# mkaspr/Vulcan

Measured on AMD Instinct MI355X. Metric: RGB-D frames/sec (integrate+raycast), 640x480 @ 5 mm voxels, higher is better.
Workload: dtype f32

## Files before the change

vulcan_amd/csrc/vk_common.hpp:

```cpp
#pragma once

#include <hip/hip_runtime.h>
#include <stdint.h>
#include <float.h>

#include "../../include/vk.h"

#define VK_CHECK(expr)                                  \
  do {                                                  \
    const hipError_t vk_e__ = (expr);                   \
    if (vk_e__ != hipSuccess)                           \
    {                                                   \
      (void)hipGetLastError();                          \
      return (int)vk_e__;                               \
    }                                                   \
  } while (0)

#define VK_REQUIRE(cond)                                \
  do {                                                  \
    if (!(cond)) return VK_ERR_ARGUMENT;                \
  } while (0)

#ifdef VK_DEBUG_SYNC
#define VK_LAUNCH_CHECK()                               \
// ... 157 lines not shown
  int16_t ox, oy, oz, pad;
  int32_t data;
  int32_t next;
};
static_assert(sizeof(Entry) == 16, "HashEntry layout");

__device__ __forceinline__ Entry load_entry(const vk_hash_entry* entries, uint32_t index)
{
  const int4 raw = reinterpret_cast<const int4*>(entries)[index];
  Entry e;
  e.ox = (int16_t)(raw.x & 0xffff);
  e.oy = (int16_t)((uint32_t)raw.x >> 16);
  e.oz = (int16_t)(raw.y & 0xffff);
  e.pad = (int16_t)((uint32_t)raw.y >> 16);
  e.data = raw.z;
  e.next = raw.w;
  return e;
}

__device__ __forceinline__ bool entry_is(const Entry& e, int bx, int by, int bz)
{
  return e.ox == (int16_t)bx && e.oy == (int16_t)by && e.oz == (int16_t)bz;
}

__device__ __forceinline__ int lane_id() { return (int)(threadIdx.x & 63); }

__device__ __forceinline__ void wave_lds_fence()
{
  __builtin_amdgcn_fence(__ATOMIC_RELEASE, "wavefront");
  __builtin_amdgcn_wave_barrier();
  __builtin_amdgcn_fence(__ATOMIC_ACQUIRE, "wavefront");
}


template <typename K>
__device__ __forceinline__ f3 normal_from_taps(const K& k, int x, int y, float depth,
    float left, float right, float up, float down)
{
  const int pad = 2;
  f3 normal = make3(0, 0, 0);
  if (depth > 0)
  {
    const f3 z0 = unproject_d(k, (x + 0) + 0.5f, (y + 0) + 0.5f, depth);
    const f3 x0 = (left == 0) ? z0 : scale3(unproject(k, (x - pad) + 0.5f, (y + 0) + 0.5f), left);
    const f3 x1 = (right == 0) ? z0 : scale3(unproject(k, (x + pad) + 0.5f, (y + 0) + 0.5f), right);
    const f3 y0 = (up == 0) ? z0 : scale3(unproject(k, (x + 0) + 0.5f, (y - pad) + 0.5f), up);
    const f3 y1 = (down == 0) ? z0 : scale3(unproject(k, (x + 0) + 0.5f, (y + pad) + 0.5f), down);
    const f3 dx = sub3(x0, x1);
    const f3 dy = sub3(y0, y1);
    if (sqnorm3(dx) > 0 && sqnorm3(dy) > 0) normal = normalized3(cross3(dy, dx));
  }
  return normal;
}

template <typename Load>
__device__ __forceinline__ float depth_or_zero(Load load, int w, int h, int x, int y)
{
  return (x >= 0 && x < w && y >= 0 && y < h) ? load(y * w + x) : 0.0f;
}

template <typename K, typename Load>
__device__ __forceinline__ f3 pixel_normal(const K& k, Load load, int w, int h, int x, int y, float depth)
{
  const int pad = 2;
  f3 normal = make3(0, 0, 0);
  if (depth > 0)
// ... 32 lines not shown
```

vulcan_amd/csrc/vk_requests.hpp:

```cpp
#pragma once

#include "vk_common.hpp"

#include <string.h>

namespace vk
{

__device__ __forceinline__ unsigned long long request_key(int type, int bx, int by, int bz)
{
  return ((unsigned long long)(uint16_t)type << 48) | ((unsigned long long)(uint16_t)(int16_t)bz << 32) |
         ((unsigned long long)(uint16_t)(int16_t)by << 16) | (unsigned long long)(uint16_t)(int16_t)bx;
}

constexpr uint8_t kTouched = 4;
__device__ __forceinline__ uint32_t band_tag(int y, int height)
{
  int band = (int)(((long long)y * VK_BANDS) / (height > 0 ? height : 1));
  band = band < 0 ? 0 : (band >= VK_BANDS ? VK_BANDS - 1 : band);
  return (uint32_t)(band + 1) << 3;
}

enum { MARK_PLAIN = 0, MARK_DEFER = 1, MARK_APPEND = 2 };

// ... 25 lines not shown
{
  return reinterpret_cast<unsigned long long*>(counters + VK_CTR_PUBLIC) + (size_t)which * VK_RETRY_SLOTS;
}
__host__ __device__ inline int* retry_slots(int32_t* counters, int which)
{
  return counters + VK_CTR_PUBLIC + 2 * 2 * VK_RETRY_SLOTS + which * VK_RETRY_KEYS;
}

__host__ __device__ inline int* posted_list(int32_t* counters)
{
  return counters + VK_CTR_PUBLIC + 2 * 2 * VK_RETRY_SLOTS + 2 * VK_RETRY_KEYS;
}
constexpr uint32_t kPostedExcess = 0x80000000u;
constexpr uint32_t kPostedBucket = 0x7fffffffu;

struct Retry
{
  int* contended;
  int* origin_seen;
  int* count;
  int* overflow;
  unsigned long long* table;
  int* slots;
  int capacity;
  int* posted;
  int* posted_tail;
  int* posted_count;
  int posted_capacity;
};

__device__ __forceinline__ void file_loser(const Retry& retry, unsigned long long key)
{
  uint32_t at = (uint32_t)((key * 0x9E3779B97F4A7C15ull) >> 40) & (uint32_t)(VK_RETRY_SLOTS - 1);
  for (int tries = 0; tries < 64; ++tries)
  {
    const unsigned long long old = atomicCAS(retry.table + at, 0ull, key);
    if (old == key) return;
    if (old == 0ull)
    {
      const int n = atomicAdd(retry.count, 1);
      if (n < retry.capacity) retry.slots[n] = (int)at;
      else __hip_atomic_store(retry.overflow, 1, __ATOMIC_RELAXED, __HIP_MEMORY_SCOPE_AGENT);
      return;
    }
    at = (at + 1) & (uint32_t)(VK_RETRY_SLOTS - 1);
  }
  __hip_atomic_store(retry.overflow, 1, __ATOMIC_RELAXED, __HIP_MEMORY_SCOPE_AGENT);
}

__device__ __forceinline__ void post_request(const vk_volume& v, uint32_t h, int type, int bx, int by, int bz,
    const Retry& retry, uint32_t tail)
{
  unsigned long long* slot = reinterpret_cast<unsigned long long*>(v.allocation_blocks) + h;
  const unsigned long long key = request_key(type, bx, by, bz);
  unsigned long long seen = __hip_atomic_load(slot, __ATOMIC_RELAXED, __HIP_MEMORY_SCOPE_AGENT);
  if (seen < key) seen = atomicMax(slot, key);
  if (retry.contended)
  {
    if (seen != 0ull && seen != key)
    {
      file_loser(retry, seen < key ? seen : key);
      if (__hip_atomic_load(retry.contended, __ATOMIC_RELAXED, __HIP_MEMORY_SCOPE_AGENT) == 0)
        __hip_atomic_store(retry.contended, 1, __ATOMIC_RELAXED, __HIP_MEMORY_SCOPE_AGENT);
    }
    if (seen == 0ull && retry.posted)
    {
// ... 27 lines not shown
  else
  {
    bool found = false;
    uint32_t index = hash_code;

    for (int guard = 0; entry.next != -1 && guard < v.excess_block_count; ++guard)
    {
      index = (uint32_t)entry.next;
      entry = load_entry(v.hash_entries, index);

      if (entry_is(entry, bx, by, bz))
      {
        mark_visible<MARK>(v, index, -1, tag);
        found = true;
        break;
      }
    }

    if (!found) post_request(v, hash_code, VK_ALLOC_EXCESS, bx, by, bz, retry, index);
  }
}

__device__ __forceinline__ int left_lane(int v)
{
  return __builtin_amdgcn_update_dpp(v, v, 0x138, 0xf, 0xf, false);
}

constexpr int kVisitSlots = 96;
constexpr int kVisitWords = 3 * kVisitSlots;
constexpr int kVisitWalkCap = 6 + 4096;

struct RequestParams
{
  vk_volume v;
  const float* depth;
  int width, height;
  Projection k;
  Rt Twd;
  const float* colors;
  const float* normals;
  Rt Tcd;
  float depth_threshold;
  float* mask;
  float4* records;
  float* normals_out;
};

template <int MARK>
__device__ __forceinline__ void request_walk(const RequestParams& P, int x, int y, const Retry& retry, int* visits)
{
  const vk_volume& v = P.v;
  const uint32_t K = (uint32_t)v.main_block_count;
  const float block_length = VK_BLOCK_RESOLUTION * v.voxel_length;
  const float truncation_length = v.truncation_length;
  const uint32_t tag = MARK == MARK_DEFER ? band_tag(y, P.height) : 0u;

  f3 direction = unproject(P.k, x + 0.5f, y + 0.5f);
  direction = xform_dir(P.Twd, direction);
  const f3 origin = make3(P.Twd.r[3], P.Twd.r[7], P.Twd.r[11]);

  float depth = 0.0f;
  if (x < P.width) depth = P.depth[y * P.width + x];
  const bool usable = x < P.width && !(depth < v.min_depth || depth > v.max_depth);

  const f3 Xwp = add3(origin, scale3(direction, depth));
  direction = normalized3(direction);
  const f3 begin = sub3(Xwp, scale3(direction, truncation_length));
  const f3 end = add3(Xwp, scale3(direction, truncation_length));

  const int step_x = (direction.x < 0) ? -1 : 1;
  const int step_y = (direction.y < 0) ? -1 : 1;
  const int step_z = (direction.z < 0) ? -1 : 1;

  const float inv_block_length = 1.0f / block_length;
  int bx = f2i(floorf(begin.x * inv_block_length));
  int by = f2i(floorf(begin.y * inv_block_length));
  int bz = f2i(floorf(begin.z * inv_block_length));
  const int ex = f2i(floorf(end.x * inv_block_length));
  const int ey = f2i(floorf(end.y * inv_block_length));
  const int ez = f2i(floorf(end.z * inv_block_length));

  const float ox = block_length * (bx + vmaxi(0, step_x)) - begin.x;
  const float oy = block_length * (by + vmaxi(0, step_y)) - begin.y;
  const float oz = block_length * (bz + vmaxi(0, step_z)) - begin.z;

  float tmax_x = ox / direction.x;
  float tmax_y = oy / direction.y;
  float tmax_z = oz / direction.z;
  if (direction.x == 0) tmax_x = (float)1E20;
  if (direction.y == 0) tmax_y = (float)1E20;
  if (direction.z == 0) tmax_z = (float)1E20;

  const float tdelta_x = (step_x * block_length) / direction.x;
  const float tdelta_y = (step_y * block_length) / direction.y;
  const float tdelta_z = (step_z * block_length) / direction.z;

  int* const list_x = visits;
  int* const list_y = visits + kVisitSlots;
  int* const list_z = visits + 2 * kVisitSlots;
  const int lane = lane_id();
  bool walking = usable;
  int listed = 0;

  for (int step = 0;; ++step)
  {
    const bool left_walking = left_lane((int)walking) != 0;
    const int left_x = left_lane(bx), left_y = left_lane(by), left_z = left_lane(bz);
    const bool fresh = walking && !(lane > 0 && left_walking && left_x == bx && left_y == by && left_z == bz);
    const unsigned long long fresh_mask = __ballot(fresh);
    const int arriving = __popcll(fresh_mask);
    const bool last = arriving == 0;

    if (listed + arriving > kVisitSlots || last)
    {
      wave_lds_fence();
      for (int first = 0; first < listed; first += 64)
      {
        const int at = first + lane;
        if (at < listed)
        {
          const int px = list_x[at], py = list_y[at], pz = list_z[at];
          const uint32_t hash_code = block_hash(px, py, pz, K);
          const Entry entry = load_entry(v.hash_entries, hash_code);
          const uint8_t byte = v.block_visibility[hash_code];
          probe_block<MARK>(v, hash_code, entry, px, py, pz, retry, (int)byte, tag);
        }
      }
      wave_lds_fence();
      listed = 0;
    }
    if (last) break;

    if (fresh)
    {
      const int at = listed + (int)__builtin_amdgcn_mbcnt_hi((uint32_t)(fresh_mask >> 32),
          __builtin_amdgcn_mbcnt_lo((uint32_t)fresh_mask, 0u));
      list_x[at] = bx; list_y[at] = by; list_z[at] = bz;
    }
    listed += arriving;

    if (walking)
    {
      if (tmax_x < tmax_y)
      {
        if (tmax_x < tmax_z) { bx += step_x; if (bx == ex + step_x) walking = false; else tmax_x += tdelta_x; }
        else                 { bz += step_z; if (bz == ez + step_z) walking = false; else tmax_z += tdelta_z; }
      }
      else
      {
        if (tmax_y < tmax_z) { by += step_y; if (by == ey + step_y) walking = false; else tmax_y += tdelta_y; }
        else                 { bz += step_z; if (bz == ez + step_z) walking = false; else tmax_z += tdelta_z; }
      }
      if (step + 1 >= kVisitWalkCap) walking = false;
    }
  }
}

template <int PREP>
struct RequestLds
{
  static constexpr int HALO = (PREP == 2) ? 2 : 1;
  static constexpr int TW = 69 + HALO, TH = 9 + HALO, TS = 72;
  static constexpr int kTileWords = PREP ? TH * TS : 0, kRowWords = PREP ? 2 * 10 * 64 : 0;
  static constexpr int kListWords = 4 * kVisitWords;
  static constexpr int kAreaWords = kTileWords + (kRowWords > kListWords ? kRowWords : kListWords);
  static constexpr int kBytes = 4 * kAreaWords;
  static_assert(!PREP || kListWords <= kRowWords, "the visit lists lie over row_min / row_max");
};
constexpr int kLdsPerCU = 160 * 1024;
constexpr int kRequestGroupsPerCU = 6;
static_assert(kRequestGroupsPerCU * RequestLds<0>::kBytes <= kLdsPerCU && kRequestGroupsPerCU * RequestLds<1>::kBytes <= kLdsPerCU &&
    kRequestGroupsPerCU * RequestLds<2>::kBytes <= kLdsPerCU, "LDS of the request pass at six workgroups per CU");

template <bool DEFER, int PREP>
__device__ __forceinline__ void requests_group(const RequestParams P, const Retry retry, const int group_x, const int group_y)
{
  const int x = group_x * 64 + (int)(threadIdx.x & 63);
  const int y = group_y * 4 + (int)(threadIdx.x >> 6);
  if (DEFER && group_x == 0 && group_y == 0 && threadIdx.x < VK_BANDS) band_counts(P.v.counters)[threadIdx.x] = 0;

  using L = RequestLds<PREP>;
  constexpr int HALO = L::HALO, TW = L::TW, TH = L::TH, TS = L::TS;
  constexpr int LOADS = (TW * TH + 255) / 256;
  __shared__ int area[L::kAreaWords];
  float* const tile = reinterpret_cast<float*>(area);
  float* const row_min = reinterpret_cast<float*>(area + L::kTileWords);
  float* const row_max = row_min + 10 * 64;
  int* const visits = area + L::kTileWords + (int)(threadIdx.x >> 6) * kVisitWords;
  float staged[LOADS] = {};
  vf3 prep_rgb = {0.0f, 0.0f, 0.0f}, prep_n = {0.0f, 0.0f, 0.0f};
  if (PREP)
  {
    const int x0 = group_x * 64 - HALO, y0 = group_y * 4 - HALO;
#pragma unroll
    for (int t = 0; t < LOADS; ++t)
    {
      const int i = (int)threadIdx.x + 256 * t;
      const int r = i / TW, c = i - r * TW;
      const int vx = x0 + c, vy = y0 + r;
      if (i < TW * TH && vx >= 0 && vx < P.width && vy >= 0 && vy < P.height) staged[t] = P.depth[vy * P.width + vx];
    }
    if (x < P.width && y < P.height)
    {
      const int index = y * P.width + x;
      prep_rgb = *reinterpret_cast<const vf3*>(P.colors + 3 * (size_t)index);
      if (PREP == 1) prep_n = *reinterpret_cast<const vf3*>(P.normals + 3 * (size_t)index);
    }
  }

  if (y < P.height) request_walk<DEFER ? MARK_DEFER : MARK_PLAIN>(P, x, y, retry, visits);

  if (PREP)
  {
#pragma unroll
    for (int t = 0; t < LOADS; ++t)
    {
      const int i = (int)threadIdx.x + 256 * t;
      if (i < TW * TH) tile[(i / TW) * TS + (i % TW)] = staged[t];
    }
    __syncthreads();
#pragma unroll
    for (int t = 0; t < 3; ++t)
    {
      const int e = (int)threadIdx.x + 256 * t;
      if (e < 10 * 64)
      {
        const float* at = tile + (HALO - 1 + (e >> 6)) * TS + (HALO + 2 + (e & 63));
        float lo = +FLT_MAX, hi = -FLT_MAX;
#pragma unroll
        for (int j = -3; j <= 3; ++j)
        {
          lo = fminf(at[j], lo);
          hi = fmaxf(at[j], hi);
        }
        row_min[e] = lo;
        row_max[e] = hi;
      }
    }
    __syncthreads();
    if (x < P.width && y < P.height)
    {
      const int index = y * P.width + x;
      const int lx = (int)(threadIdx.x & 63) + HALO, ly = (int)(threadIdx.x >> 6) + HALO;
      f3 normal = make3(prep_n.x, prep_n.y, prep_n.z);
      if (PREP == 2)
      {
        normal = normal_from_taps(P.k, x, y, tile[ly * TS + lx], tile[ly * TS + lx - 2], tile[ly * TS + lx + 2],
            tile[(ly - 2) * TS + lx], tile[(ly + 2) * TS + lx]);
        P.normals_out[3 * (size_t)index + 0] = normal.x;
        P.normals_out[3 * (size_t)index + 1] = normal.y;
        P.normals_out[3 * (size_t)index + 2] = normal.z;
      }
      const f3 Xcn = xform_dir(P.Tcd, normal);
      float m = 0.0f;
      if (light_color_usable(prep_rgb.x, prep_rgb.y, prep_rgb.z))
      {
        const int first = (int)(threadIdx.x >> 6) * 64 + (int)(threadIdx.x & 63);
        float dmin = +FLT_MAX, dmax = -FLT_MAX;
#pragma unroll
        for (int i = 0; i < 7; ++i)
        {
          dmin = fminf(row_min[first + 64 * i], dmin);
          dmax = fmaxf(row_max[first + 64 * i], dmax);
        }
        m = (dmax - dmin <= P.depth_threshold) ? 1.0f : 0.0f;
      }
      P.mask[index] = m;
      P.records[index] = make_float4(Xcn.x, Xcn.y, Xcn.z, m);
    }
  }
}


constexpr int kArrivalMaxWorkgroups = 65535;

inline int posted_capacity()
{
  const int n = vk_hook(VK_HOOK_POSTED_CAPACITY);
  return (n >= 0 && n < VK_POSTED_SLOTS) ? n : VK_POSTED_SLOTS;
}

inline int retry_capacity()
{
  const int n = vk_hook(VK_HOOK_RETRY_CAPACITY);
  return (n > 0 && n < VK_RETRY_KEYS) ? n : VK_RETRY_KEYS;
}

inline bool set_view_unfused(const vk_volume* v)
{
  const bool unfused = vk_hook(VK_HOOK_SET_VIEW_UNFUSED) == 1;
  return unfused || ((long long)v->main_block_count + v->excess_block_count) / 1024 + 16 > kArrivalMaxWorkgroups;
}

inline bool prep_rides(const vk_light_prep* prep, const vk_frame* frame)
{
  return prep && prep->mask && prep->records && frame->color && frame->normals && frame->content_id != 0 &&
      (long long)frame->width * frame->height <= (long long)prep->capacity &&
      (reinterpret_cast<uintptr_t>(prep->records) & 15) == 0 &&
      (frame->color_width <= 0 || frame->color_width == frame->width) &&
      (frame->color_height <= 0 || frame->color_height == frame->height);
}

inline void prep_note_made(vk_light_prep* prep, const vk_frame* frame)
{
  prep->depth = frame->depth;
  prep->color = frame->color;
  prep->normals = frame->normals;
  prep->width = frame->width;
  prep->height = frame->height;
  prep->depth_to_color = frame->depth_to_color;
  prep->content_id = frame->content_id;
  prep->prepared_threshold = prep->depth_threshold;
  prep->valid = 1;
  prep->normals_out = nullptr;
}

inline int build_request_pass(RequestParams& P, Retry& retry, const vk_volume* v, const float* depth, int width, int height,
    const vk_projection* projection, const vk_transform* Twd, const vk_frame* prep_frame, const vk_light_prep* prep, bool fused)
{
  P.v = *v;
  P.depth = depth;
  P.width = width;
  P.height = height;
  P.k = make_projection(*projection);
  P.Twd = make_rt(Twd->m);
  P.colors = P.normals = nullptr;
  P.Tcd = P.Twd;
  P.depth_threshold = 0.0f;
  P.mask = nullptr;
  P.records = nullptr;
  P.normals_out = nullptr;
  memset(&retry, 0, sizeof(retry));
  if (fused)
  {
    retry.contended = v->counters + VK_CTR_CONTENDED;
    retry.origin_seen = v->counters + VK_CTR_ORIGIN_SEEN;
    retry.count = v->counters + VK_CTR_RETRY_COUNT;
    retry.overflow = v->counters + VK_CTR_RETRY_OVERFLOW;
    retry.table = retry_table(v->counters, 0);
    retry.slots = retry_slots(v->counters, 0);
    retry.capacity = retry_capacity();
    if (!set_view_unfused(v))
    {
      retry.posted = posted_list(v->counters);
      retry.posted_tail = posted_list(v->counters) + VK_POSTED_SLOTS;
      retry.posted_count = v->counters + VK_CTR_POSTED;
      retry.posted_capacity = posted_capacity();
    }
  }
  if (!(prep && prep_frame)) return 0;
  P.colors = prep_frame->color;
  P.normals = prep_frame->normals;
  P.Tcd = make_rt(prep_frame->depth_to_color.m);
  P.depth_threshold = prep->depth_threshold;
  P.mask = prep->mask;
  P.records = reinterpret_cast<float4*>(prep->records);
  P.normals_out = prep->normals_out;
  return prep->normals_out ? 2 : 1;
}

}
```

vulcan_amd/csrc/vk_trace.hip:

```cpp
#include "vk_bounds.hpp"
#include "vk_raycast.hpp"
#include "vk_requests.hpp"

using namespace vk;

namespace
{


constexpr int kPatchThreads = 256;

__global__ __launch_bounds__(kPatchThreads) void compute_patches_kernel(PatchParams P)
{
  __shared__ int wave_total[kPatchThreads / 64];
  __shared__ int block_base;

  const int block_count = P.block_count_dev ? min(*P.block_count_dev, P.block_count) : P.block_count;
  const int index = blockIdx.x * kPatchThreads + threadIdx.x;
  const int lane = lane_id();
  const int wave = threadIdx.x >> 6;

  BlockRect r;
  r.count = 0;
  r.gx = r.gy = 0;
// ... 236 lines not shown
{
  if (threadIdx.x == 0)
  {
    const int first = vmaxi(group_y * 4 - 2, 0) >> 3, last = vmini(group_y * 4 + 5, P.image_height - 1) >> 3;
    int polls = 0;
    bool late = false;
    for (int row = first; row <= last && !late; ++row)
      while ((int)(__hip_atomic_load(&P.rows_done[row * kNormalRowStride], __ATOMIC_RELAXED, __HIP_MEMORY_SCOPE_AGENT) - P.rows_target) < 0)
      {
        if (++polls > P.normal_polls) { late = true; break; }
        __builtin_amdgcn_s_sleep(32);
      }
    *expired = late ? 1 : 0;
    if (late)
    {
      __hip_atomic_store(P.late_dev, P.late_tag, __ATOMIC_RELAXED, __HIP_MEMORY_SCOPE_AGENT);
      if (P.late_host) __hip_atomic_store(P.late_host, (int32_t)P.late_tag, __ATOMIC_RELAXED, __HIP_MEMORY_SCOPE_SYSTEM);
    }
  }
  __syncthreads();
  if (*expired) return;
  const int x = group_x * 64 + (threadIdx.x & 63);
  const int y = group_y * 4 + (threadIdx.x >> 6);
  if (x >= P.image_width || y >= P.image_height) return;
  const auto written = [depths = P.depths](int i) { return __hip_atomic_load(&depths[i], __ATOMIC_RELAXED, __HIP_MEMORY_SCOPE_AGENT); };
  const f3 normal = pixel_normal(P.k, written, P.image_width, P.image_height, x, y,
      depth_or_zero(written, P.image_width, P.image_height, x, y));
  const int output = y * P.image_width + x;
  normals[3 * output + 0] = normal.x;
  normals[3 * output + 1] = normal.y;
  normals[3 * output + 2] = normal.z;
}

template <bool POOL32, int PREP>
__global__ __launch_bounds__(256) __attribute__((amdgpu_waves_per_eu(VK_TR_WAVES))) void trace_and_request_kernel(PointParams P,
    RequestParams R, Retry retry, int trace_groups, int request_groups_x, int request_groups, float* normals)
{
  __shared__ int4 directories[4][kDirWords];
  __shared__ int normals_expired;
  static_assert(kRequestGroupsPerCU * (int)(sizeof(directories) + sizeof(int) + RequestLds<PREP>::kBytes) <= kLdsPerCU,
      "LDS of the raycast + request launch at six workgroups per CU");
  if ((int)blockIdx.x < trace_groups)
  {
    __builtin_amdgcn_s_setprio(2);
    points_group<POOL32, 4>(P, (int)blockIdx.x, trace_groups, directories);
    return;
  }
  const int g = (int)blockIdx.x - trace_groups;
  if (g < request_groups)
  {
    requests_group<true, PREP>(R, retry, g % request_groups_x, g / request_groups_x);
    return;
  }
  const int n = g - request_groups, normal_groups_x = (P.image_width + 63) / 64;
  normals_group(P, normals, n % normal_groups_x, n / normal_groups_x, &normals_expired);
}


__global__ __launch_bounds__(256) void compute_normals_kernel(const float* __restrict__ depths,
    vk_projection k, float* __restrict__ normals, int image_width, int image_height)
{
  const int x = blockIdx.x * 64 + (threadIdx.x & 63);
  const int y = blockIdx.y * 4 + (threadIdx.x >> 6);
  if (x >= image_width || y >= image_height) return;

  const f3 normal = pixel_normal(k, plain_depths{depths}, image_width, image_height, x, y, depths[y * image_width + x]);

  const int output = y * image_width + x;
  normals[3 * output + 0] = normal.x;
  normals[3 * output + 1] = normal.y;
  normals[3 * output + 2] = normal.z;
}

__global__ __launch_bounds__(256) void filter_depths_kernel(int image_width, int image_height,
    const float* __restrict__ src, float* __restrict__ dst)
{
  const int x = blockIdx.x * 64 + (threadIdx.x & 63);
  const int y = blockIdx.y * 4 + (threadIdx.x >> 6);
  if (x >= image_width || y >= image_height) return;

  const int pad = 3;
  const float d0 = src[y * image_width + x];
  float dn = 0;
  float w = 0;

  for (int i = -pad; i <= pad; ++i)
// ... 18 lines not shown
{
  const int cells = P.bounds_width * P.bounds_height;

  if (partials && cells <= kBoundsMaxCells)
  {
    hipLaunchKernelGGL(block_bounds_partial_kernel, dim3(kBoundsGroups), dim3(kBoundsThreads), 0, s, P, partials);
    VK_LAUNCH_CHECK();
    if (merge)
    {
      hipLaunchKernelGGL(merge_bounds_kernel, dim3((cells + 255) / 256), dim3(256), 0, s, partials,
          reinterpret_cast<float2*>(bounds), cells);
      VK_LAUNCH_CHECK();
    }
    return VK_OK;
  }

  hipLaunchKernelGGL(reset_bounds_kernel, dim3((cells + 255) / 256), dim3(256), 0, s,
      reinterpret_cast<float2*>(bounds), cells);
  VK_LAUNCH_CHECK();
  if (P.block_count == 0) return VK_OK;
  P.bounds = bounds;
  int blocks = (P.block_count + 255) / 256;
  if (blocks > kCUs * 4) blocks = kCUs * 4;
  hipLaunchKernelGGL(block_bounds_kernel, dim3(blocks), dim3(256), 0, s, P);
  VK_LAUNCH_CHECK();
  return VK_OK;
}

int launch_points(const vk_hash_entry* entries, const vk_voxel* voxels, const float* bounds,
    const float2* partials, int block_count, float block_length, float voxel_length, float trunc_length,
    const vk_transform* Twc, const vk_projection* projection, float* depths, float* colors,
    int image_width, int image_height, int bounds_width, int bounds_height, unsigned long long pool_bytes,
    hipStream_t s, float* normals = nullptr, uint32_t* rows_done = nullptr, uint32_t rows_target = 0,
    const RequestParams* next_requests = nullptr, const Retry* next_retry = nullptr, int next_prep = 0,
    int32_t* late_host = nullptr, int normal_polls = kNormalWaitPolls, uint32_t late_tag = 1)
{
  PointParams P;
  P.late_tag = late_tag ? late_tag : 1u;
  P.entries = entries;
  P.voxels = voxels;
  P.bounds = bounds;
  P.partials = partials;
  P.bounds_out = reinterpret_cast<float2*>(const_cast<float*>(bounds));
  P.K = (uint32_t)block_count;
  P.block_length = block_length;
  P.voxel_length = voxel_length;
  P.trunc_length = trunc_length;
  P.inv_block_length = 1.0 / (double)block_length;
  P.inv_voxel_length = 1.0 / (double)voxel_length;
  P.touched = nullptr;
  P.march_steps = nullptr;
  P.trip_log = nullptr;
  P.trip_log_passes = 0;
  P.rows_done = (normals && rows_done && next_requests) ? rows_done : nullptr;
  P.rows_target = rows_target;
  P.late_dev = P.rows_done ? P.rows_done + kNormalRows * kNormalRowStride : nullptr;
  P.late_host = late_host;
  P.normal_polls = normal_polls;
  P.Twc = make_rt(Twc->m);
  P.Tcw = make_rt(Twc->inv);
  P.k = make_projection(*projection);
  P.depths = depths;
  P.colors = colors;
  P.image_width = image_width;
  P.image_height = image_height;
  P.bounds_width = bounds_width;
  P.bounds_height = bounds_height;
  const bool pool32 = pool_bytes <= 0xffffffffull;
  if (next_requests)
  {
    const int tiles16 = ((image_width + 15) / 16) * ((image_height + 15) / 16);
    int chunk16 = (tiles16 + 7) / 8;
    chunk16 = 2 * ((chunk16 + 1) / 2);
    const int trace_groups = 8 * chunk16;
    const int normal_groups = P.rows_done ? ((image_width + 63) / 64) * ((image_height + 3) / 4) : 0;
    const int gx = (next_requests->width + 63) / 64, gy = (next_requests->height + 3) / 4;
    const dim3 grid2(trace_groups + gx * gy + normal_groups);
    float* fused_normals = P.rows_done ? normals : nullptr;
#define VK_LAUNCH_TR(POOL, PREP) hipLaunchKernelGGL((trace_and_request_kernel<POOL, PREP>), grid2, dim3(256), 0, s, P, *next_requests, *next_retry, trace_groups, gx, gx * gy, fused_normals)
    if (pool32) { if (next_prep == 2) VK_LAUNCH_TR(true, 2); else if (next_prep == 1) VK_LAUNCH_TR(true, 1); else VK_LAUNCH_TR(true, 0); }
    else { if (next_prep == 2) VK_LAUNCH_TR(false, 2); else if (next_prep == 1) VK_LAUNCH_TR(false, 1); else VK_LAUNCH_TR(false, 0); }
#undef VK_LAUNCH_TR
    VK_LAUNCH_CHECK();
    return VK_OK;
  }
  const int tiles = ((image_width + kPointsTile - 1) / kPointsTile) * ((image_height + kPointsTile - 1) / kPointsTile);
  int chunk = (tiles + 7) / 8;
  chunk = 2 * ((chunk + 1) / 2);
  const dim3 grid(8 * chunk);
  if (pool32)
    hipLaunchKernelGGL(compute_points_kernel<true>, grid, dim3(kPointsWaves * 64), 0, s, P);
  else
    hipLaunchKernelGGL(compute_points_kernel<false>, grid, dim3(kPointsWaves * 64), 0, s, P);
  VK_LAUNCH_CHECK();
  return VK_OK;
}

int launch_normals(const float* depths, const vk_projection* projection, float* normals,
    int image_width, int image_height, hipStream_t s)
{
  const dim3 grid((image_width + 63) / 64, (image_height + 3) / 4);
  hipLaunchKernelGGL(compute_normals_kernel, grid, dim3(256), 0, s, depths, *projection, normals,
      image_width, image_height);
  VK_LAUNCH_CHECK();
  return VK_OK;
}

}

extern "C" {

int vk_trace_compute_patches(const int32_t* indices, const vk_hash_entry* entries,
// ... 111 lines not shown
           v->voxel_length, v->truncation_length, &frame->depth_to_world, &frame->depth_projection,
           out_depth, out_color, frame->width, frame->height, bounds_width, bounds_height,
           (unsigned long long)max_count * VK_BLOCK_VOXELS * sizeof(vk_voxel), s)) != VK_OK)
    return rc;

  return launch_normals(out_depth, &frame->depth_projection, out_normals, frame->width, frame->height, s);
}

static uint32_t* normals_counters(const vk_view_bounds* ahead)
{
  const int cells = ahead->bounds_width * ahead->bounds_height;
  if (cells > kBoundsMaxCells) return nullptr;
  return reinterpret_cast<uint32_t*>(ahead->scratch + 2 * (size_t)cells * (1 + kBoundsGroups));
}

static int normals_repair(vk_view_bounds* ahead, hipStream_t s)
{
  if (ahead->counted_stream && ahead->counted_stream != (const void*)s)
    VK_CHECK(hipStreamSynchronize(reinterpret_cast<hipStream_t>(const_cast<void*>(ahead->counted_stream))));
  uint32_t* counters = normals_counters(ahead);
  if (counters) VK_CHECK(hipMemsetAsync(counters, 0, (kNormalRows * kNormalRowStride + kNormalLateWords) * sizeof(uint32_t), s));
  if (ahead->late_host) __atomic_store_n(ahead->late_host, 0, __ATOMIC_RELAXED);
  ahead->trace_launches = 0;
  if (ahead->last_depths && ahead->last_normals && ahead->last_width > 0 && ahead->last_height > 0)
  {
    const int rc = launch_normals(ahead->last_depths, &ahead->last_projection, ahead->last_normals, ahead->last_width,
        ahead->last_height, s);
    if (rc != VK_OK) return rc;
  }
  return VK_ERR_TIMEOUT;
}

static int trace_ahead(const vk_volume* v, const vk_frame* frame, vk_view_bounds* ahead, float* out_depth,
    float* out_color, float* out_normals, void* stream, const RequestParams* next_requests, const Retry* next_retry, int next_prep)
{
  VK_REQUIRE(v && frame && ahead && ahead->scratch && out_depth && out_color && (out_normals || !next_requests));
  VK_REQUIRE(v->hash_entries && v->voxels && v->visible_blocks && v->counters);
  VK_REQUIRE(ahead->bounds_width > 0 && ahead->bounds_height > 0);
  hipStream_t s = vk_s(stream);
  if (ahead->late_host && __atomic_load_n(ahead->late_host, __ATOMIC_RELAXED) != 0)
  {
    VK_CHECK(hipStreamSynchronize(s));
    return normals_repair(ahead, s);
  }
  const float block_length = VK_BLOCK_RESOLUTION * v->voxel_length;
  const int cells = ahead->bounds_width * ahead->bounds_height;
  float* bounds = ahead->scratch;
  float2* partials = (cells <= kBoundsMaxCells) ? reinterpret_cast<float2*>(bounds) + cells : nullptr;
  int rc;

  if (!(partials && view_matches(ahead, v, frame)))
  {
    ahead->valid = 0;
    PatchParams P;
    if ((rc = view_patch_params(P, v, frame, ahead)) != VK_OK) return rc;
    if ((rc = launch_block_bounds(P, bounds, partials, false, s)) != VK_OK) return rc;
    if (partials) view_record(ahead, v, frame);
  }

  const int rows = 2 * ((frame->height + 15) / 16), waves_per_row = 2 * ((frame->width + 15) / 16);
  const bool normals_ride = next_requests && out_normals && partials && rows <= kNormalRows;
  uint32_t* rows_done = nullptr;
  uint32_t rows_target = 0;
  if (normals_ride)
  {
    rows_done = reinterpret_cast<uint32_t*>(bounds + 2 * (size_t)cells * (1 + kBoundsGroups));
    if (ahead->counted_scratch != bounds || ahead->counted_width != frame->width || ahead->counted_height != frame->height ||
        ahead->counted_stream != stream)
    {
      VK_CHECK(hipMemsetAsync(rows_done, 0, (kNormalRows * kNormalRowStride + kNormalLateWords) * sizeof(uint32_t), s));
      ahead->counted_scratch = bounds;
      ahead->counted_width = frame->width;
      ahead->counted_height = frame->height;
      ahead->counted_stream = stream;
      ahead->trace_launches = 0;
    }
    rows_target = (ahead->trace_launches + 1u) * (uint32_t)waves_per_row;
  }
  int normal_polls = kNormalWaitPolls;
  if (normals_ride && vk_hook_take(VK_HOOK_FORCE_NORMALS_EXPIRY) == 1)
  {
    rows_target += 0x40000000u;
    normal_polls = 0;
  }
  if ((rc = launch_points(v->hash_entries, v->voxels, bounds, partials, v->main_block_count, block_length,
           v->voxel_length, v->truncation_length, &frame->depth_to_world, &frame->depth_projection,
           out_depth, out_color, frame->width, frame->height, ahead->bounds_width, ahead->bounds_height,
           (unsigned long long)(v->main_block_count + v->excess_block_count) * VK_BLOCK_VOXELS * sizeof(vk_voxel), s,
           normals_ride ? out_normals : nullptr, rows_done, rows_target, next_requests, next_retry, next_prep,
           ahead->late_host, normal_polls, (ahead->trace_launches + 1u) & 0x7fffffffu)) != VK_OK)
    return rc;
  if (normals_ride)
  {
    ++ahead->trace_launches;
    ahead->last_depths = out_depth;
    ahead->last_normals = out_normals;
    ahead->last_width = frame->width;
    ahead->last_height = frame->height;
    ahead->last_projection = frame->depth_projection;
    return VK_OK;
  }
  ahead->last_depths = nullptr;
  ahead->last_normals = nullptr;
  if (!out_normals) return VK_OK;
  return launch_normals(out_depth, &frame->depth_projection, out_normals, frame->width, frame->height, s);
}

int vk_trace_ahead(const vk_volume* v, const vk_frame* frame, vk_view_bounds* ahead, float* out_depth,
    float* out_color, float* out_normals, void* stream)
{
  return trace_ahead(v, frame, ahead, out_depth, out_color, out_normals, stream, nullptr, nullptr, 0);
}

int vk_trace_ahead_requests(const vk_volume* v, const vk_frame* view, vk_view_bounds* ahead, float* out_depth,
    float* out_color, float* out_normals, const vk_frame* next, vk_light_prep* next_prep, vk_requests_ahead* requests,
    void* stream)
{
  VK_REQUIRE(v && next && requests);
  if (requests->valid == 1) return VK_ERR_ARGUMENT;
  requests->valid = 0;
  const bool ride = prep_rides(next_prep, next);
  const bool possible = next->depth && next->width > 0 && next->height > 0 && next->content_id != 0 && v->counters &&
      v->allocation_types && v->allocation_blocks && v->block_visibility &&
      !(next_prep && next_prep->normals_out && (!ride || next_prep->normals_out != next->normals));
  if (!possible) return vk_trace_ahead(v, view, ahead, out_depth, out_color, out_normals, stream);
  RequestParams R;
  Retry retry;
  const int with_prep = build_request_pass(R, retry, v, next->depth, next->width, next->height, &next->depth_projection,
      &next->depth_to_world, ride ? next : nullptr, ride ? next_prep : nullptr, true);
  if (next_prep) next_prep->valid = 0;
  const int rc = trace_ahead(v, view, ahead, out_depth, out_color, out_normals, stream, &R, &retry, with_prep);
  if (rc != VK_OK) return rc;
  if (ride) prep_note_made(next_prep, next);
  requests->counters = v->counters;
  requests->depth = next->depth;
  requests->prep = ride ? next_prep : nullptr;
  requests->width = next->width;
  requests->height = next->height;
  requests->depth_projection = next->depth_projection;
  requests->depth_to_world = next->depth_to_world;
  requests->content_id = next->content_id;
  requests->normals_made = with_prep == 2 ? 1 : 0;
  requests->pose_on_device = 0;
  requests->valid = 1;
  return VK_OK;
}

int vk_trace_ahead_pyramid(const vk_volume* v, const vk_frame* frame, vk_view_bounds* ahead, float* out_depth, float* out_color,
    float* out_normals, const vk_icp_view* next, float* pyramid, vk_pyramid_ahead* built, void* stream)
{
  VK_REQUIRE(v && frame && next && pyramid && built && out_normals);
  built->valid = 0;
  VK_REQUIRE(next->depths && next->normals && next->width > 0 && next->height > 0);
  VK_REQUIRE(((frame->width | frame->height | next->width | next->height) & 1) == 0);
  built->pad_ = 0;
  return vk_trace_ahead(v, frame, ahead, out_depth, out_color, out_normals, stream);
}

int vk_trace_normals_settle(vk_view_bounds* ahead, void* stream)
{
  VK_REQUIRE(ahead && ahead->scratch && ahead->bounds_width > 0 && ahead->bounds_height > 0);
  hipStream_t s = vk_s(stream);
  VK_CHECK(hipStreamSynchronize(s));
  bool late = false;
// ... 12 lines not shown
```

vulcan_amd/csrc/vk_volume.hip:

```cpp
#include "vk_common.hpp"
#include "vk_requests.hpp"

#include <stdlib.h>
#include <string.h>

using namespace vk;

namespace
{


__global__ __launch_bounds__(256) void fill_voxels_kernel(float4* __restrict__ voxels4, size_t n4)
{
  const size_t stride = (size_t)gridDim.x * blockDim.x;
  for (size_t j = (size_t)blockIdx.x * blockDim.x + threadIdx.x; j < n4; j += stride)
  {
    const size_t d = j * 4;
    float4 v;
    v.x = ((d + 0) % 5 == 0) ? 1.0f : 0.0f;
    v.y = ((d + 1) % 5 == 0) ? 1.0f : 0.0f;
    v.z = ((d + 2) % 5 == 0) ? 1.0f : 0.0f;
    v.w = ((d + 3) % 5 == 0) ? 1.0f : 0.0f;
    voxels4[j] = v;
  }
// ... 19 lines not shown

  if (i < VK_CTR_PUBLIC)
  {
    int value = 0;
    if (i == VK_CTR_EXCESS_PTR) value = v.main_block_count;
    if (i == VK_CTR_VOXEL_PTR) value = max_count - 1;
    v.counters[i] = value;
  }
}


__global__ __launch_bounds__(256) void reset_visibility_kernel(uint8_t* __restrict__ vis, int count)
{
  const int words = count >> 2;
  const int i = blockIdx.x * blockDim.x + threadIdx.x;

  if (i < words)
  {
    uint32_t w = reinterpret_cast<uint32_t*>(vis)[i];
    const uint32_t is_true = (w >> 1) & 0x01010101u;
    w &= ~(is_true * 0x3u);
    reinterpret_cast<uint32_t*>(vis)[i] = w;
  }

  if (i < (count & 3))
  {
    const int j = (words << 2) + i;
    if (vis[j] == VK_VISIBILITY_TRUE) vis[j] = VK_VISIBILITY_UNKNOWN;
  }
}


template <bool DEFER, int PREP>
__global__ __launch_bounds__(256) __attribute__((amdgpu_waves_per_eu(5))) void create_requests_kernel(RequestParams P, Retry retry)
{
  requests_group<DEFER, PREP>(P, retry, (int)blockIdx.x, (int)blockIdx.y);
}

template <int PREP>
__global__ __launch_bounds__(256) __attribute__((amdgpu_waves_per_eu(5))) void create_requests_at_kernel(RequestParams P, Retry retry,
    const vk_transform* __restrict__ pose)
{
#pragma unroll
  for (int r = 0; r < 3; ++r)
#pragma unroll
    for (int c = 0; c < 4; ++c) P.Twd.r[r * 4 + c] = pose->m[c * 4 + r];
  requests_group<true, PREP>(P, retry, (int)blockIdx.x, (int)blockIdx.y);
}


constexpr int kHandleThreads = 256;
constexpr int kHandlePerGroup = 4 * kHandleThreads;

__device__ __forceinline__ void block_sum2(int& a, int& b, int* lds)
{
#pragma unroll
  for (int d = 32; d >= 1; d >>= 1)
  {
    a += __shfl_xor(a, d);
    b += __shfl_xor(b, d);
  }
  const int wave = threadIdx.x >> 6;
  if (lane_id() == 0) { lds[2 * wave] = a; lds[2 * wave + 1] = b; }
  __syncthreads();
  a = 0;
  b = 0;
#pragma unroll
  for (int w = 0; w < kHandleThreads / 64; ++w) { a += lds[2 * w]; b += lds[2 * w + 1]; }
  __syncthreads();
}

__device__ __forceinline__ void count_flags(uint32_t w, int& n_all, int& n_excess)
{
  n_all += __popc((w | (w >> 1)) & 0x01010101u);
  n_excess += __popc((w >> 1) & 0x01010101u);
}

__device__ __forceinline__ void handle_group(const vk_volume& v, int group, int groups, int zero_visible,
    int deferred_reset, int* dropped_now)
{
// ... 995 lines not shown
  handle_visibility_body(P);
}

__global__ __launch_bounds__(kHandleThreads) void handle_visibility_at_kernel(FusedParams P, const vk_transform* __restrict__ pose)
{
#pragma unroll
  for (int r = 0; r < 3; ++r)
#pragma unroll
    for (int c = 0; c < 4; ++c) P.vis.Tdw.r[r * 4 + c] = pose->inv[c * 4 + r];
  handle_visibility_body(P);
}

int check_volume(const vk_volume* v)
{
  if (!v) return VK_ERR_ARGUMENT;
  if (!v->voxels || !v->hash_entries || !v->free_voxel_blocks || !v->allocation_types ||
      !v->allocation_blocks || !v->block_visibility || !v->visible_blocks || !v->counters)
    return VK_ERR_ARGUMENT;
  if (v->main_block_count <= 0 || v->excess_block_count < 0) return VK_ERR_ARGUMENT;
  if (!(v->voxel_length > 0) || !(v->truncation_length > 0)) return VK_ERR_ARGUMENT;
  if ((reinterpret_cast<uintptr_t>(v->counters) & 7) || (reinterpret_cast<uintptr_t>(v->allocation_blocks) & 7) || (reinterpret_cast<uintptr_t>(v->hash_entries) & 15) ||
      (reinterpret_cast<uintptr_t>(v->voxels) & 15) || (reinterpret_cast<uintptr_t>(v->block_visibility) & 3) ||
      (reinterpret_cast<uintptr_t>(v->allocation_types) & 15))
    return VK_ERR_ARGUMENT;
  return VK_OK;
}

int launch_create_requests(const vk_volume* v, const float* depth, int width, int height,
    const vk_projection* projection, const vk_transform* Twd, bool deferred_reset, hipStream_t s,
    const vk_frame* prep_frame = nullptr, const vk_light_prep* prep = nullptr, bool fused = false,
    const vk_transform* pose_dev = nullptr)
{
  RequestParams P;
  Retry retry;
  const int with_prep = build_request_pass(P, retry, v, depth, width, height, projection, Twd, prep_frame, prep, fused);
  const dim3 grid((width + 63) / 64, (height + 3) / 4);
  if (pose_dev)
  {
    if (with_prep == 2 || !deferred_reset) return VK_ERR_UNSUPPORTED;
    if (with_prep == 1) hipLaunchKernelGGL((create_requests_at_kernel<1>), grid, dim3(256), 0, s, P, retry, pose_dev);
    else hipLaunchKernelGGL((create_requests_at_kernel<0>), grid, dim3(256), 0, s, P, retry, pose_dev);
    VK_LAUNCH_CHECK();
    return VK_OK;
  }
  if (with_prep == 2) hipLaunchKernelGGL((create_requests_kernel<true, 2>), grid, dim3(256), 0, s, P, retry);
  else if (with_prep == 1) hipLaunchKernelGGL((create_requests_kernel<true, 1>), grid, dim3(256), 0, s, P, retry);
  else if (deferred_reset) hipLaunchKernelGGL((create_requests_kernel<true, 0>), grid, dim3(256), 0, s, P, retry);
  else hipLaunchKernelGGL((create_requests_kernel<false, 0>), grid, dim3(256), 0, s, P, retry);
  VK_LAUNCH_CHECK();
  return VK_OK;
}

int launch_update_visibility(const vk_volume* v, int width, int height,
    const vk_projection* projection, const float* Tdw_m, int finish, bool deferred_reset, hipStream_t s)
{
  VisibilityParams P;
  P.v = *v;
  P.finish_handle = finish;
  P.deferred_reset = deferred_reset ? 1 : 0;
  P.width = width;
  P.height = height;
  P.k = *projection;
  P.Tdw = make_rt(Tdw_m);
  const int count = v->main_block_count + v->excess_block_count;
  hipLaunchKernelGGL(update_visibility_kernel, dim3((count + kVisThreads - 1) / kVisThreads),
      dim3(kVisThreads), 0, s, P);
  VK_LAUNCH_CHECK();
  return VK_OK;
}

int launch_reset_visibility(const vk_volume* v, hipStream_t s)
{
  const int count = v->main_block_count + v->excess_block_count;
  const int threads = (count >> 2) > 4 ? (count >> 2) : 4;
  hipLaunchKernelGGL(reset_visibility_kernel, dim3((threads + 255) / 256), dim3(256), 0, s,
      v->block_visibility, count);
  VK_LAUNCH_CHECK();
  return VK_OK;
}

}
// ... 250 lines not shown
```

Baseline: 8347.

## Read request-pass parameters lazily from kernarg segment to cut SGPR pressure

Request kernels now take one packed argument struct and read fields on demand through the kernarg segment pointer, with an asm barrier so loads are not hoisted. Parameters are regrouped into walk, probe and prep sections, so the volume and retry state load only when a wave flushes its visit list. Block length, its inverse and the depth limits are precomputed on the host. The aim is lower scalar register pressure and fewer spills in the fused trace+request kernel and the standalone request kernels, at the cost of repeated scalar loads from kernarg memory.

```diff
diff --git a/vulcan_amd/csrc/vk_common.hpp b/vulcan_amd/csrc/vk_common.hpp
--- a/vulcan_amd/csrc/vk_common.hpp
+++ b/vulcan_amd/csrc/vk_common.hpp
@@ -213,6 +213,21 @@
   __builtin_amdgcn_fence(__ATOMIC_ACQUIRE, "wavefront");
 }
 
+
+template <typename T>
+using karg = const __attribute__((address_space(4))) T*;
+
+template <typename T>
+__device__ __forceinline__ karg<T> kernel_arguments()
+{
+  return (karg<T>)__builtin_amdgcn_kernarg_segment_ptr();
+}
+template <typename T>
+__device__ __forceinline__ const T& arguments_now(karg<T> p)
+{
+  asm volatile("" : "+s"(p));
+  return *(const T*)p;
+}
 
 template <typename K>
 __device__ __forceinline__ f3 normal_from_taps(const K& k, int x, int y, float depth,
diff --git a/vulcan_amd/csrc/vk_requests.hpp b/vulcan_amd/csrc/vk_requests.hpp
--- a/vulcan_amd/csrc/vk_requests.hpp
+++ b/vulcan_amd/csrc/vk_requests.hpp
@@ -81,6 +81,7 @@
 __device__ __forceinline__ void file_loser(const Retry& retry, unsigned long long key)
 {
   uint32_t at = (uint32_t)((key * 0x9E3779B97F4A7C15ull) >> 40) & (uint32_t)(VK_RETRY_SLOTS - 1);
+#pragma unroll 1
   for (int tries = 0; tries < 64; ++tries)
   {
     const unsigned long long old = atomicCAS(retry.table + at, 0ull, key);
@@ -174,36 +175,47 @@
 
 struct RequestParams
 {
-  vk_volume v;
-  const float* depth;
-  int width, height;
-  Projection k;
-  Rt Twd;
+  struct Walk
+  {
+    const float* depth;
+    int width, height;
+    Projection k;
+    Rt Twd;
+    float truncation_length, min_depth, max_depth;
+    float block_length, inv_block_length;
+  } walk;
+  struct Probe
+  {
+    vk_volume v;
+    Retry retry;
+  } probe;
   const float* colors;
   const float* normals;
-  Rt Tcd;
-  float depth_threshold;
-  float* mask;
-  float4* records;
-  float* normals_out;
+  struct Prep
+  {
+    Rt Tcd;
+    float depth_threshold;
+    float* mask;
+    float4* records;
+    float* normals_out;
+  } prep;
 };
 
 template <int MARK>
-__device__ __forceinline__ void request_walk(const RequestParams& P, int x, int y, const Retry& retry, int* visits)
-{
-  const vk_volume& v = P.v;
-  const uint32_t K = (uint32_t)v.main_block_count;
-  const float block_length = VK_BLOCK_RESOLUTION * v.voxel_length;
-  const float truncation_length = v.truncation_length;
-  const uint32_t tag = MARK == MARK_DEFER ? band_tag(y, P.height) : 0u;
+__device__ __forceinline__ void request_walk(const RequestParams::Walk& P, const Rt& Twd, karg<RequestParams::Probe> probe,
+    int x, int y, int* visits)
+{
+  const float block_length = P.block_length;
+  const float truncation_length = P.truncation_length;
+  const uint32_t tag = MARK == MARK_DEFER ? band_tag(__builtin_amdgcn_readfirstlane(y), P.height) : 0u;
 
   f3 direction = unproject(P.k, x + 0.5f, y + 0.5f);
-  direction = xform_dir(P.Twd, direction);
-  const f3 origin = make3(P.Twd.r[3], P.Twd.r[7], P.Twd.r[11]);
+  direction = xform_dir(Twd, direction);
+  const f3 origin = make3(Twd.r[3], Twd.r[7], Twd.r[11]);
 
   float depth = 0.0f;
   if (x < P.width) depth = P.depth[y * P.width + x];
-  const bool usable = x < P.width && !(depth < v.min_depth || depth > v.max_depth);
+  const bool usable = x < P.width && !(depth < P.min_depth || depth > P.max_depth);
 
   const f3 Xwp = add3(origin, scale3(direction, depth));
   direction = normalized3(direction);
@@ -214,7 +226,7 @@
   const int step_y = (direction.y < 0) ? -1 : 1;
   const int step_z = (direction.z < 0) ? -1 : 1;
 
-  const float inv_block_length = 1.0f / block_length;
+  const float inv_block_length = P.inv_block_length;
   int bx = f2i(floorf(begin.x * inv_block_length));
   int by = f2i(floorf(begin.y * inv_block_length));
   int bz = f2i(floorf(begin.z * inv_block_length));
@@ -256,6 +268,10 @@
     if (listed + arriving > kVisitSlots || last)
     {
       wave_lds_fence();
+      const RequestParams::Probe S = arguments_now(probe);
+      const vk_volume& v = S.v;
+      const Retry& retry = S.retry;
+      const uint32_t K = (uint32_t)v.main_block_count;
       for (int first = 0; first < listed; first += 64)
       {
         const int at = first + lane;
@@ -315,11 +331,13 @@
     kRequestGroupsPerCU * RequestLds<2>::kBytes <= kLdsPerCU, "LDS of the request pass at six workgroups per CU");
 
 template <bool DEFER, int PREP>
-__device__ __forceinline__ void requests_group(const RequestParams P, const Retry retry, const int group_x, const int group_y)
+__device__ __forceinline__ void requests_group(karg<RequestParams> args, const int group_x, const int group_y, const Rt* pose = nullptr)
 {
   const int x = group_x * 64 + (int)(threadIdx.x & 63);
   const int y = group_y * 4 + (int)(threadIdx.x >> 6);
-  if (DEFER && group_x == 0 && group_y == 0 && threadIdx.x < VK_BANDS) band_counts(P.v.counters)[threadIdx.x] = 0;
+  if (DEFER && group_x == 0 && group_y == 0 && threadIdx.x < VK_BANDS)
+    band_counts(arguments_now(&args->probe.v.counters))[threadIdx.x] = 0;
+  const RequestParams::Walk P = arguments_now(&args->walk);
 
   using L = RequestLds<PREP>;
   constexpr int HALO = L::HALO, TW = L::TW, TH = L::TH, TS = L::TS;
@@ -345,19 +363,23 @@
     if (x < P.width && y < P.height)
     {
       const int index = y * P.width + x;
-      prep_rgb = *reinterpret_cast<const vf3*>(P.colors + 3 * (size_t)index);
-      if (PREP == 1) prep_n = *reinterpret_cast<const vf3*>(P.normals + 3 * (size_t)index);
-    }
-  }
-
-  if (y < P.height) request_walk<DEFER ? MARK_DEFER : MARK_PLAIN>(P, x, y, retry, visits);
+      prep_rgb = *reinterpret_cast<const vf3*>(arguments_now(&args->colors) + 3 * (size_t)index);
+      if (PREP == 1) prep_n = *reinterpret_cast<const vf3*>(arguments_now(&args->normals) + 3 * (size_t)index);
+    }
+  }
+
+  if (__builtin_amdgcn_readfirstlane(y) < P.height)
+    request_walk<DEFER ? MARK_DEFER : MARK_PLAIN>(P, pose ? *pose : P.Twd, &args->probe, x, y, visits);
 
   if (PREP)
   {
+    int thread = (int)threadIdx.x;
+    asm volatile("" : "+v"(thread));
+    thread &= 255;
 #pragma unroll
     for (int t = 0; t < LOADS; ++t)
     {
-      const int i = (int)threadIdx.x + 256 * t;
+      const int i = thread + 256 * t;
       if (i < TW * TH) tile[(i / TW) * TS + (i % TW)] = staged[t];
     }
     __syncthreads();
@@ -380,20 +402,24 @@
       }
     }
     __syncthreads();
-    if (x < P.width && y < P.height)
-    {
-      const int index = y * P.width + x;
+    const RequestParams& A = arguments_now(args);
+    const int width = A.walk.width, height = A.walk.height;
+    const RequestParams::Prep Q = A.prep;
+    if (x < width && y < height)
+    {
+      const int index = y * width + x;
       const int lx = (int)(threadIdx.x & 63) + HALO, ly = (int)(threadIdx.x >> 6) + HALO;
       f3 normal = make3(prep_n.x, prep_n.y, prep_n.z);
       if (PREP == 2)
       {
-        normal = normal_from_taps(P.k, x, y, tile[ly * TS + lx], tile[ly * TS + lx - 2], tile[ly * TS + lx + 2],
+        const Projection k = A.walk.k;
+        normal = normal_from_taps(k, x, y, tile[ly * TS + lx], tile[ly * TS + lx - 2], tile[ly * TS + lx + 2],
             tile[(ly - 2) * TS + lx], tile[(ly + 2) * TS + lx]);
-        P.normals_out[3 * (size_t)index + 0] = normal.x;
-        P.normals_out[3 * (size_t)index + 1] = normal.y;
-        P.normals_out[3 * (size_t)index + 2] = normal.z;
-      }
-      const f3 Xcn = xform_dir(P.Tcd, normal);
+        Q.normals_out[3 * (size_t)index + 0] = normal.x;
+        Q.normals_out[3 * (size_t)index + 1] = normal.y;
+        Q.normals_out[3 * (size_t)index + 2] = normal.z;
+      }
+      const f3 Xcn = xform_dir(Q.Tcd, normal);
       float m = 0.0f;
       if (light_color_usable(prep_rgb.x, prep_rgb.y, prep_rgb.z))
       {
@@ -405,10 +431,10 @@
           dmin = fminf(row_min[first + 64 * i], dmin);
           dmax = fmaxf(row_max[first + 64 * i], dmax);
         }
-        m = (dmax - dmin <= P.depth_threshold) ? 1.0f : 0.0f;
-      }
-      P.mask[index] = m;
-      P.records[index] = make_float4(Xcn.x, Xcn.y, Xcn.z, m);
+        m = (dmax - dmin <= Q.depth_threshold) ? 1.0f : 0.0f;
+      }
+      Q.mask[index] = m;
+      Q.records[index] = make_float4(Xcn.x, Xcn.y, Xcn.z, m);
     }
   }
 }
@@ -457,21 +483,29 @@
   prep->normals_out = nullptr;
 }
 
-inline int build_request_pass(RequestParams& P, Retry& retry, const vk_volume* v, const float* depth, int width, int height,
+inline int build_request_pass(RequestParams& R, const vk_volume* v, const float* depth, int width, int height,
     const vk_projection* projection, const vk_transform* Twd, const vk_frame* prep_frame, const vk_light_prep* prep, bool fused)
 {
-  P.v = *v;
-  P.depth = depth;
-  P.width = width;
-  P.height = height;
-  P.k = make_projection(*projection);
-  P.Twd = make_rt(Twd->m);
-  P.colors = P.normals = nullptr;
-  P.Tcd = P.Twd;
+  RequestParams::Walk& W = R.walk;
+  W.depth = depth;
+  W.width = width;
+  W.height = height;
+  W.k = make_projection(*projection);
+  W.Twd = make_rt(Twd->m);
+  W.block_length = VK_BLOCK_RESOLUTION * v->voxel_length;
+  W.inv_block_length = 1.0f / W.block_length;
+  W.truncation_length = v->truncation_length;
+  W.min_depth = v->min_depth;
+  W.max_depth = v->max_depth;
+  R.probe.v = *v;
+  R.colors = R.normals = nullptr;
+  RequestParams::Prep& P = R.prep;
+  P.Tcd = W.Twd;
   P.depth_threshold = 0.0f;
   P.mask = nullptr;
   P.records = nullptr;
   P.normals_out = nullptr;
+  Retry& retry = R.probe.retry;
   memset(&retry, 0, sizeof(retry));
   if (fused)
   {
@@ -491,8 +525,8 @@
     }
   }
   if (!(prep && prep_frame)) return 0;
-  P.colors = prep_frame->color;
-  P.normals = prep_frame->normals;
+  R.colors = prep_frame->color;
+  R.normals = prep_frame->normals;
   P.Tcd = make_rt(prep_frame->depth_to_color.m);
   P.depth_threshold = prep->depth_threshold;
   P.mask = prep->mask;
diff --git a/vulcan_amd/csrc/vk_trace.hip b/vulcan_amd/csrc/vk_trace.hip
--- a/vulcan_amd/csrc/vk_trace.hip
+++ b/vulcan_amd/csrc/vk_trace.hip
@@ -292,26 +292,40 @@
   normals[3 * output + 2] = normal.z;
 }
 
+struct TraceRequestParams
+{
+  int trace_groups, request_groups_x, request_groups;
+  float* normals;
+  PointParams P;
+  RequestParams R;
+};
+
 template <bool POOL32, int PREP>
-__global__ __launch_bounds__(256) __attribute__((amdgpu_waves_per_eu(VK_TR_WAVES))) void trace_and_request_kernel(PointParams P,
-    RequestParams R, Retry retry, int trace_groups, int request_groups_x, int request_groups, float* normals)
+__global__ __launch_bounds__(256) __attribute__((amdgpu_waves_per_eu(VK_TR_WAVES))) void trace_and_request_kernel(TraceRequestParams)
 {
   __shared__ int4 directories[4][kDirWords];
   __shared__ int normals_expired;
   static_assert(kRequestGroupsPerCU * (int)(sizeof(directories) + sizeof(int) + RequestLds<PREP>::kBytes) <= kLdsPerCU,
       "LDS of the raycast + request launch at six workgroups per CU");
+  const karg<TraceRequestParams> args = kernel_arguments<TraceRequestParams>();
+  const int trace_groups = args->trace_groups;
   if ((int)blockIdx.x < trace_groups)
   {
     __builtin_amdgcn_s_setprio(2);
+    const PointParams P = arguments_now(&args->P);
     points_group<POOL32, 4>(P, (int)blockIdx.x, trace_groups, directories);
     return;
   }
   const int g = (int)blockIdx.x - trace_groups;
+  const int request_groups = args->request_groups;
   if (g < request_groups)
   {
-    requests_group<true, PREP>(R, retry, g % request_groups_x, g / request_groups_x);
+    const int request_groups_x = args->request_groups_x;
+    requests_group<true, PREP>(&args->R, g % request_groups_x, g / request_groups_x);
     return;
   }
+  const PointParams P = arguments_now(&args->P);
+  float* const normals = arguments_now(&args->normals);
   const int n = g - request_groups, normal_groups_x = (P.image_width + 63) / 64;
   normals_group(P, normals, n % normal_groups_x, n / normal_groups_x, &normals_expired);
 }
@@ -396,7 +410,7 @@
     const vk_transform* Twc, const vk_projection* projection, float* depths, float* colors,
     int image_width, int image_height, int bounds_width, int bounds_height, unsigned long long pool_bytes,
     hipStream_t s, float* normals = nullptr, uint32_t* rows_done = nullptr, uint32_t rows_target = 0,
-    const RequestParams* next_requests = nullptr, const Retry* next_retry = nullptr, int next_prep = 0,
+    const RequestParams* next_requests = nullptr, int next_prep = 0,
     int32_t* late_host = nullptr, int normal_polls = kNormalWaitPolls, uint32_t late_tag = 1)
 {
   PointParams P;
@@ -438,10 +452,16 @@
     chunk16 = 2 * ((chunk16 + 1) / 2);
     const int trace_groups = 8 * chunk16;
     const int normal_groups = P.rows_done ? ((image_width + 63) / 64) * ((image_height + 3) / 4) : 0;
-    const int gx = (next_requests->width + 63) / 64, gy = (next_requests->height + 3) / 4;
+    const int gx = (next_requests->walk.width + 63) / 64, gy = (next_requests->walk.height + 3) / 4;
     const dim3 grid2(trace_groups + gx * gy + normal_groups);
-    float* fused_normals = P.rows_done ? normals : nullptr;
-#define VK_LAUNCH_TR(POOL, PREP) hipLaunchKernelGGL((trace_and_request_kernel<POOL, PREP>), grid2, dim3(256), 0, s, P, *next_requests, *next_retry, trace_groups, gx, gx * gy, fused_normals)
+    TraceRequestParams A;
+    A.trace_groups = trace_groups;
+    A.request_groups_x = gx;
+    A.request_groups = gx * gy;
+    A.normals = P.rows_done ? normals : nullptr;
+    A.P = P;
+    A.R = *next_requests;
+#define VK_LAUNCH_TR(POOL, PREP) hipLaunchKernelGGL((trace_and_request_kernel<POOL, PREP>), grid2, dim3(256), 0, s, A)
     if (pool32) { if (next_prep == 2) VK_LAUNCH_TR(true, 2); else if (next_prep == 1) VK_LAUNCH_TR(true, 1); else VK_LAUNCH_TR(true, 0); }
     else { if (next_prep == 2) VK_LAUNCH_TR(false, 2); else if (next_prep == 1) VK_LAUNCH_TR(false, 1); else VK_LAUNCH_TR(false, 0); }
 #undef VK_LAUNCH_TR
@@ -619,7 +639,7 @@
 }
 
 static int trace_ahead(const vk_volume* v, const vk_frame* frame, vk_view_bounds* ahead, float* out_depth,
-    float* out_color, float* out_normals, void* stream, const RequestParams* next_requests, const Retry* next_retry, int next_prep)
+    float* out_color, float* out_normals, void* stream, const RequestParams* next_requests, int next_prep)
 {
   VK_REQUIRE(v && frame && ahead && ahead->scratch && out_depth && out_color && (out_normals || !next_requests));
   VK_REQUIRE(v->hash_entries && v->voxels && v->visible_blocks && v->counters);
@@ -674,7 +694,7 @@
            v->voxel_length, v->truncation_length, &frame->depth_to_world, &frame->depth_projection,
            out_depth, out_color, frame->width, frame->height, ahead->bounds_width, ahead->bounds_height,
            (unsigned long long)(v->main_block_count + v->excess_block_count) * VK_BLOCK_VOXELS * sizeof(vk_voxel), s,
-           normals_ride ? out_normals : nullptr, rows_done, rows_target, next_requests, next_retry, next_prep,
+           normals_ride ? out_normals : nullptr, rows_done, rows_target, next_requests, next_prep,
            ahead->late_host, normal_polls, (ahead->trace_launches + 1u) & 0x7fffffffu)) != VK_OK)
     return rc;
   if (normals_ride)
@@ -696,7 +716,7 @@
 int vk_trace_ahead(const vk_volume* v, const vk_frame* frame, vk_view_bounds* ahead, float* out_depth,
     float* out_color, float* out_normals, void* stream)
 {
-  return trace_ahead(v, frame, ahead, out_depth, out_color, out_normals, stream, nullptr, nullptr, 0);
+  return trace_ahead(v, frame, ahead, out_depth, out_color, out_normals, stream, nullptr, 0);
 }
 
 int vk_trace_ahead_requests(const vk_volume* v, const vk_frame* view, vk_view_bounds* ahead, float* out_depth,
@@ -712,11 +732,10 @@
       !(next_prep && next_prep->normals_out && (!ride || next_prep->normals_out != next->normals));
   if (!possible) return vk_trace_ahead(v, view, ahead, out_depth, out_color, out_normals, stream);
   RequestParams R;
-  Retry retry;
-  const int with_prep = build_request_pass(R, retry, v, next->depth, next->width, next->height, &next->depth_projection,
+  const int with_prep = build_request_pass(R, v, next->depth, next->width, next->height, &next->depth_projection,
       &next->depth_to_world, ride ? next : nullptr, ride ? next_prep : nullptr, true);
   if (next_prep) next_prep->valid = 0;
-  const int rc = trace_ahead(v, view, ahead, out_depth, out_color, out_normals, stream, &R, &retry, with_prep);
+  const int rc = trace_ahead(v, view, ahead, out_depth, out_color, out_normals, stream, &R, with_prep);
   if (rc != VK_OK) return rc;
   if (ride) prep_note_made(next_prep, next);
   requests->counters = v->counters;
diff --git a/vulcan_amd/csrc/vk_volume.hip b/vulcan_amd/csrc/vk_volume.hip
--- a/vulcan_amd/csrc/vk_volume.hip
+++ b/vulcan_amd/csrc/vk_volume.hip
@@ -75,20 +75,21 @@
 
 
 template <bool DEFER, int PREP>
-__global__ __launch_bounds__(256) __attribute__((amdgpu_waves_per_eu(5))) void create_requests_kernel(RequestParams P, Retry retry)
-{
-  requests_group<DEFER, PREP>(P, retry, (int)blockIdx.x, (int)blockIdx.y);
+__global__ __launch_bounds__(256) __attribute__((amdgpu_waves_per_eu(5))) void create_requests_kernel(RequestParams)
+{
+  requests_group<DEFER, PREP>(kernel_arguments<RequestParams>(), (int)blockIdx.x, (int)blockIdx.y);
 }
 
 template <int PREP>
-__global__ __launch_bounds__(256) __attribute__((amdgpu_waves_per_eu(5))) void create_requests_at_kernel(RequestParams P, Retry retry,
+__global__ __launch_bounds__(256) __attribute__((amdgpu_waves_per_eu(5))) void create_requests_at_kernel(RequestParams,
     const vk_transform* __restrict__ pose)
 {
+  Rt Twd;
 #pragma unroll
   for (int r = 0; r < 3; ++r)
 #pragma unroll
-    for (int c = 0; c < 4; ++c) P.Twd.r[r * 4 + c] = pose->m[c * 4 + r];
-  requests_group<true, PREP>(P, retry, (int)blockIdx.x, (int)blockIdx.y);
+    for (int c = 0; c < 4; ++c) Twd.r[r * 4 + c] = pose->m[c * 4 + r];
+  requests_group<true, PREP>(kernel_arguments<RequestParams>(), (int)blockIdx.x, (int)blockIdx.y, &Twd);
 }
 
 
@@ -1150,21 +1151,20 @@
     const vk_transform* pose_dev = nullptr)
 {
   RequestParams P;
-  Retry retry;
-  const int with_prep = build_request_pass(P, retry, v, depth, width, height, projection, Twd, prep_frame, prep, fused);
+  const int with_prep = build_request_pass(P, v, depth, width, height, projection, Twd, prep_frame, prep, fused);
   const dim3 grid((width + 63) / 64, (height + 3) / 4);
   if (pose_dev)
   {
     if (with_prep == 2 || !deferred_reset) return VK_ERR_UNSUPPORTED;
-    if (with_prep == 1) hipLaunchKernelGGL((create_requests_at_kernel<1>), grid, dim3(256), 0, s, P, retry, pose_dev);
-    else hipLaunchKernelGGL((create_requests_at_kernel<0>), grid, dim3(256), 0, s, P, retry, pose_dev);
+    if (with_prep == 1) hipLaunchKernelGGL((create_requests_at_kernel<1>), grid, dim3(256), 0, s, P, pose_dev);
+    else hipLaunchKernelGGL((create_requests_at_kernel<0>), grid, dim3(256), 0, s, P, pose_dev);
     VK_LAUNCH_CHECK();
     return VK_OK;
   }
-  if (with_prep == 2) hipLaunchKernelGGL((create_requests_kernel<true, 2>), grid, dim3(256), 0, s, P, retry);
-  else if (with_prep == 1) hipLaunchKernelGGL((create_requests_kernel<true, 1>), grid, dim3(256), 0, s, P, retry);
-  else if (deferred_reset) hipLaunchKernelGGL((create_requests_kernel<true, 0>), grid, dim3(256), 0, s, P, retry);
-  else hipLaunchKernelGGL((create_requests_kernel<false, 0>), grid, dim3(256), 0, s, P, retry);
+  if (with_prep == 2) hipLaunchKernelGGL((create_requests_kernel<true, 2>), grid, dim3(256), 0, s, P);
+  else if (with_prep == 1) hipLaunchKernelGGL((create_requests_kernel<true, 1>), grid, dim3(256), 0, s, P);
+  else if (deferred_reset) hipLaunchKernelGGL((create_requests_kernel<true, 0>), grid, dim3(256), 0, s, P);
+  else hipLaunchKernelGGL((create_requests_kernel<false, 0>), grid, dim3(256), 0, s, P);
   VK_LAUNCH_CHECK();
   return VK_OK;
 }
```

New measurement: 8266. About the same (-1.0%).
